# EricLBuehler/mistral.rs

Measured on AMD Instinct MI355X. Metric: decode_tokens_per_sec, higher is better.
Workload: dtype q4_k/q6_k weights x q8_k activations (int8 dot, f32 accumulate: the reference CPU path's arithmetic); 1 GPU; Llama-3-8B GGUF Q4_K_M, TP=1, 512 prefill / 1599 decode, batch 1, paged KV bf16 (block 32); parallelism=tp1

## Files before the change

### mistral.rs_amd/csrc/ext_gemm_qi.hip

```cpp
#include "dec_core2.cuh"
#include <stdio.h>
#include <stdlib.h>
#include <algorithm>
#include <type_traits>

namespace mrs {
namespace qi {
using namespace mrs::dec2;

typedef _Float16 h2 __attribute__((ext_vector_type(2)));
typedef _Float16 h8 __attribute__((ext_vector_type(8)));
typedef float f16v __attribute__((ext_vector_type(16)));
typedef float f2 __attribute__((ext_vector_type(2)));

constexpr int REC_Q4K = 4096 + 512 + 128, REC_Q6K = 8192 + 512 + 128, REC_Q5K = REC_Q6K;
__host__ __device__ constexpr int rec_bytes_qi(int type) { return type == T_Q4_K ? REC_Q4K : REC_Q6K; }
__host__ __device__ inline bool qi_type(int t) { return t == T_Q4_K || t == T_Q5_K || t == T_Q6_K || t == T_Q8_0; }
__host__ __device__ inline size_t qi_tensor_bytes(int type, long long n, long long k) { return (size_t)((n + 31) / 32) * (size_t)(k / 256) * rec_bytes_qi(type); }

__host__ __device__ constexpr int perm8(int jj) { return jj == 1 ? 2 : jj == 2 ? 1 : jj == 5 ? 6 : jj == 6 ? 5 : jj; }

template <int TYPE>
__global__ void __launch_bounds__(256) qi_repack_kernel(const uint8_t *__restrict__ src, uint8_t *__restrict__ dst, long long n, int K, long long total) {
  const long long i = (long long)blockIdx.x * 256 + threadIdx.x;
  if (i >= total) return;
  const int S = K / 256, lane = (int)(i & 63);
  const long long ps = i >> 6;
  const int sb = (int)(ps % S);
  const long long panel = ps / S, row = panel * 32 + (lane & 31);
  const int hf = lane >> 5;
  const bool have = row < n;
  uint8_t *rec = dst + (size_t)ps * rec_bytes_qi(TYPE);
  alignas(16) uint8_t buf[16];
  if constexpr (TYPE == T_Q4_K) {
    const uint8_t *b = src + ((size_t)row * S + sb) * 144, *qs = b + 16;
    for (int c = 0; c < 4; ++c) {
      for (int k = 0; k < 8; ++k) { buf[k] = have ? qs[32 * c + 8 * hf + k] : 0; buf[8 + k] = have ? qs[32 * c + 16 + 8 * hf + k] : 0; }
      *(v4u *)(rec + ((size_t)c * 64 + lane) * 16) = *(const v4u *)buf;
    }
    if (hf == 0) {
      const int nn = lane & 31;
      for (int g = 0; g < 8; ++g) {
        uint8_t sc = 0, mn = 0;
        if (have) {
          const uint8_t *p = b + 4;
          if (g < 4) { sc = p[g] & 63; mn = p[g + 4] & 63; } else { sc = (p[g + 4] & 15) | ((p[g - 4] >> 6) << 4); mn = (p[g + 4] >> 4) | ((p[g] >> 6) << 4); }
// ... 25 lines not shown
      *(uint32_t *)(rec + 8704 + (size_t)nn * 4) = have ? ((uint32_t)b[0] | ((uint32_t)b[1] << 8) | ((uint32_t)b[2] << 16) | ((uint32_t)b[3] << 24)) : 0u;
    }
  } else if constexpr (TYPE == T_Q8_0) {
    const uint8_t *b = src + ((size_t)row * S + sb) * 272;
    for (int g = 0; g < 8; ++g) {
      for (int k = 0; k < 16; ++k) buf[k] = have ? b[34 * g + 2 + 16 * hf + k] : 0;
      *(v4u *)(rec + ((size_t)g * 64 + lane) * 16) = *(const v4u *)buf;
    }
    if (hf == 0) {
      const int nn = lane & 31;
      for (int g = 0; g < 8; ++g) { buf[2 * g] = have ? b[34 * g] : 0; buf[2 * g + 1] = have ? b[34 * g + 1] : 0; }
      *(v4u *)(rec + 8192 + (size_t)nn * 16) = *(const v4u *)buf;
      *(uint32_t *)(rec + 8704 + (size_t)nn * 4) = 0u;
    }
  } else {
    const uint8_t *b = src + ((size_t)row * S + sb) * 210, *ql = b, *qh = b + 128;
    auto q6 = [&](int e) { const int hh = e / 128, pos = e % 32, qt = (e % 128) / 32, ii = hh * 64 + pos + (qt % 2) * 32;
                           const int lo = qt < 2 ? (ql[ii] & 15) : (ql[ii] >> 4), hi = (qh[hh * 32 + pos] >> (qt * 2)) & 3; return lo | (hi << 4); };
    for (int g = 0; g < 8; ++g) {
      for (int k = 0; k < 8; ++k) { buf[k] = have ? (uint8_t)q6((2 * g) * 16 + 8 * hf + k) : 32; buf[8 + k] = have ? (uint8_t)q6((2 * g + 1) * 16 + 8 * hf + k) : 32; }
      *(v4u *)(rec + ((size_t)g * 64 + lane) * 16) = *(const v4u *)buf;
    }
    if (hf == 0) {
      const int nn = lane & 31;
      for (int k = 0; k < 16; ++k) buf[k] = have ? b[192 + k] : 0;
      *(v4u *)(rec + 8192 + (size_t)nn * 16) = *(const v4u *)buf;
      *(uint32_t *)(rec + 8704 + (size_t)nn * 4) = have ? ((uint32_t)b[208] | ((uint32_t)b[209] << 8)) : 0u;
    }
  }
}

struct QuantArgs {
  const float *x, *x2; int ldx; const float *norm_w; float eps; int K, T;
  _Float16 *qf; float *yd; _Float16 *bsf;
  float *xtmp;
  int mode;
};
template <bool GLU>
__global__ void __launch_bounds__(NT) qi_quantize_kernel(const QuantArgs a) {
  extern __shared__ __attribute__((aligned(16))) char smem[];
  __shared__ float red[8];
  const int tid = tid_opaque(), t = blockIdx.x, K = a.K, S = K / 256;
  const float *xr = a.x + (size_t)t * a.ldx;
  if constexpr (GLU) {
    float *dst = a.xtmp + (size_t)t * K;
    const float *ur = a.x2 + (size_t)t * a.ldx;
    for (int e = tid * 4; e < K; e += NT * 4) {
      const float4 g = *(const float4 *)(xr + e), u = *(const float4 *)(ur + e);
      *(float4 *)(dst + e) = make_float4(silu_engine(g.x) * u.x, silu_engine(g.y) * u.y, silu_engine(g.z) * u.z, silu_engine(g.w) * u.w);
    }
    __syncthreads();
    xr = dst;
  }
  const int qw = __builtin_amdgcn_readfirstlane(tid >> 6);
  const ActRegs<1> pre = act_issue_all<1>(xr, (unsigned)K * 4u, a.norm_w, K, qw);
  act_finish_all<1>(smem, red, pre, xr, K, a.norm_w, a.eps, K, a.mode, qw);
  __syncthreads();
  const Act act = act_view(smem, K, 1, a.mode);
  if (a.mode == ACT_Q80) {
    int8_t *q8 = (int8_t *)a.qf;
    float *yd8 = (float *)a.bsf;
    for (int gi = tid; gi < S * 16; gi += NT) {
      const int sb = gi >> 4, ch = gi & 15;
      *(v4u *)(q8 + ((size_t)sb * a.T + t) * 256 + ch * 16) = *(const v4u *)(act.q + act.qoff(sb) + ch * 16);
    }
    for (int i = tid; i < S * 8; i += NT) {
      const int sb = i >> 3, b = i & 7;
      yd8[((size_t)sb * 8 + b) * a.T + t] = act.d[(size_t)sb * act.dw + b];
    }
    return;
  }
  for (int gi = tid; gi < S * 32; gi += NT) {
    const int sb = gi >> 5, g8 = gi & 31;
    const int8_t *q = (const int8_t *)(act.q + act.qoff(sb) + g8 * 8);
    h8 o;
#pragma unroll
    for (int jj = 0; jj < 8; ++jj) o[jj] = (_Float16)(float)q[perm8(jj)];
    *(h8 *)(a.qf + ((size_t)sb * a.T + t) * 256 + g8 * 8) = o;
  }
  for (int i = tid; i < S * 16; i += NT) {
    const int sb = i >> 4, r = i & 15;
    a.bsf[((size_t)sb * a.T + t) * 16 + r] = (_Float16)(float)act.bs[(size_t)sb * ACT_BS + r];
  }
  for (int sb = tid; sb < S; sb += NT) a.yd[(size_t)sb * a.T + t] = act.d[sb];
}

struct GemmArgs {
  const uint8_t *w; unsigned w_bytes; int type, N, K, T;
  const _Float16 *qf; const float *yd; const _Float16 *bsf;
  float *out; int ldo; int accumulate;
  float *part; int ksplit;
  const int *win;
};
constexpr int TN = 128, TT = 128;
constexpr int GT = 512;
constexpr int LDS_ACT = TT * 512, LDS_YD = TT * 4, LDS_BS = TT * 32;
constexpr int LDS_BUF = LDS_ACT + LDS_YD + LDS_BS;
constexpr int LDS_TOTAL = 2 * LDS_BUF;

#ifndef MRS_GLDS16
#define MRS_GLDS16(gptr, lbase) __builtin_amdgcn_global_load_lds((const __attribute__((address_space(1))) void *)(gptr), (__attribute__((address_space(3))) void *)(lbase), 16, 0, 0)
#define MRS_GLDS4(gptr, lbase) __builtin_amdgcn_global_load_lds((const __attribute__((address_space(1))) void *)(gptr), (__attribute__((address_space(3))) void *)(lbase), 4, 0, 0)
#endif
#ifndef MRS_WAIT_VMCNT0
#define MRS_WAIT_VMCNT0() asm volatile("s_waitcnt vmcnt(0)" ::: "memory")
#endif

__device__ __forceinline__ h2 as_h2(unsigned v) { return __builtin_bit_cast(h2, v); }
__device__ __forceinline__ h8 mk_h8(h2 a, h2 b, h2 c, h2 d) { h8 r; r[0] = a[0]; r[1] = a[1]; r[2] = b[0]; r[3] = b[1]; r[4] = c[0]; r[5] = c[1]; r[6] = d[0]; r[7] = d[1]; return r; }
__device__ __forceinline__ h2 pkfma(h2 x, h2 s, h2 c) { return __builtin_elementwise_fma(x, s, c); }
__device__ __forceinline__ h2 magic(unsigned v, unsigned mask) { return as_h2((v & mask) | 0x64006400u); }

template <int TYPE>
__global__ void __launch_bounds__(GT) gemm_qi_kernel(const GemmArgs a) {
  extern __shared__ __attribute__((aligned(16))) char smem[];
  const int tid = tid_opaque(), lane = tid & 63, wave = __builtin_amdgcn_readfirstlane(tid >> 6);
  const int nn = lane & 31, hf = lane >> 5;
  const int n0 = blockIdx.x * TN;
  const int tbeg = a.win ? __builtin_amdgcn_readfirstlane(a.win[0]) : 0, tend = a.win ? __builtin_amdgcn_readfirstlane(a.win[1]) : a.T;
  const int t0 = tbeg + blockIdx.y * TT;
  if (t0 >= tend) return;
  const int wn = wave & 3, wt = wave >> 2;
  const int S = a.K / 256, Cs = (S + 3) / 4;
  const __amdgpu_buffer_rsrc_t rw = __builtin_amdgcn_make_buffer_rsrc((void *)a.w, (short)0, (int)a.w_bytes, 0x00020000);
  constexpr int REC = rec_bytes_qi(TYPE), NPC = TYPE == T_Q4_K ? 4 : 8;
  struct WRegs { v4u q[NPC]; v4u hs; unsigned hd; };
  const unsigned panel = (unsigned)((n0 + wn * 32) >> 5);
  auto load_w = [&](WRegs &wr, int sb) {
    const unsigned rec = (panel * (unsigned)S + (unsigned)sb) * (unsigned)REC;
#pragma unroll
    for (int c = 0; c < NPC; ++c) wr.q[c] = __builtin_amdgcn_raw_buffer_load_b128(rw, rec + (unsigned)(c * 64 + lane) * 16u, 0, 0);
    wr.hs = __builtin_amdgcn_raw_buffer_load_b128(rw, rec + (unsigned)(NPC * 1024) + (unsigned)nn * 16u, 0, 0);
    wr.hd = __builtin_amdgcn_raw_buffer_load_b32(rw, rec + (unsigned)(NPC * 1024 + 512) + (unsigned)nn * 4u, 0, 0);
  };
  const int tlast = tend - 1 - t0;
  auto stage = [&](int sb, int buf) {
    char *base = smem + buf * LDS_BUF;
    const char *gq = (const char *)a.qf + ((size_t)sb * a.T + t0) * 512;
#pragma unroll
    for (int i = 0; i < 8; ++i) {
      const int pair = wave * 8 + i;
      const int tr = 2 * pair + hf, trc = min(tr, tlast);
      MRS_GLDS16(gq + (size_t)trc * 512 + (((lane & 31) ^ (tr & 31)) << 4), base + pair * 1024);
    }
    if (wave < 2) {
      const int tr = wave * 64 + lane;
      MRS_GLDS4((const char *)a.yd + ((size_t)sb * a.T + t0 + min(tr, tlast)) * 4, base + LDS_ACT + wave * 256);
    } else if (wave < 6) {
      const int i = wave - 2, tr = i * 32 + (lane >> 1);
      MRS_GLDS16((const char *)a.bsf + ((size_t)sb * a.T + t0 + min(tr, tlast)) * 32 + (lane & 1) * 16, base + LDS_ACT + LDS_YD + i * 1024);
    }
  };
  f16v run[2], pend[2];
#pragma unroll
  for (int tt = 0; tt < 2; ++tt)
#pragma unroll
    for (int v = 0; v < 16; ++v) { run[tt][v] = 0.f; pend[tt][v] = 0.f; }
  WRegs wr, wnx;
  const int sb_first = a.ksplit > 1 ? (int)blockIdx.z * ((a.K / 256 + 3) / 4) : 0;
  if (sb_first < a.K / 256) { load_w(wr, sb_first); stage(sb_first, sb_first & 1); }
  const int trow = wt * 64 + nn;
  int aoff[16];
#pragma unroll
  for (int r = 0; r < 16; ++r) aoff[r] = trow * 512 + (((2 * r + hf) ^ nn) << 4);
  const int sb_begin = a.ksplit > 1 ? (int)blockIdx.z * Cs : 0, sb_end = a.ksplit > 1 ? min(S, sb_begin + Cs) : S;
  if (sb_begin >= sb_end) {
    if (a.ksplit > 1) {
      const int n = n0 + wn * 32 + nn;
#pragma unroll
      for (int tt = 0; tt < 2; ++tt)
#pragma unroll
        for (int v = 0; v < 16; ++v) {
          const int t = t0 + wt * 64 + tt * 32 + 8 * (v >> 2) + 4 * hf + (v & 3);
          if (n < a.N && t < tend) a.part[((size_t)blockIdx.z * a.T + t) * a.N + n] = 0.f;
        }
    }
    return;
  }
  for (int sb = sb_begin; sb < sb_end; ++sb) {
    const int buf = sb & 1;
    MRS_WAIT_VMCNT0();
    __syncthreads();
    if (sb + 1 < sb_end) { stage(sb + 1, buf ^ 1); load_w(wnx, sb + 1); }
    const char *act_s = smem + buf * LDS_BUF;
    const float *yd_s = (const float *)(act_s + LDS_ACT);
    const char *bs_s = act_s + LDS_ACT + LDS_YD;
    f16v X[2], X2[2];
#pragma unroll
    for (int tt = 0; tt < 2; ++tt)
#pragma unroll
      for (int v = 0; v < 16; ++v) { X[tt][v] = 0.f; X2[tt][v] = 0.f; }
    constexpr bool RECOMP = TYPE == T_Q5_K;
    int nnv = nn;
    if constexpr (RECOMP) MRS_OPAQUE_TID(nnv);
    auto act_frag = [&](int tt, int run_i) -> h8 {
      if constexpr (RECOMP) return *(const h8 *)(act_s + trow * 512 + (((2 * run_i + hf) ^ nnv) << 4) + tt * (32 * 512));
      else return *(const h8 *)(act_s + aoff[run_i] + tt * (32 * 512));
    };
    const bool cfirst = (sb % Cs) == 0;
    const f2 keep2 = cfirst ? f2{0.f, 0.f} : f2{1.f, 1.f};
    if constexpr (TYPE == T_Q4_K) {
      unsigned mg = 0x64006400u;
      MRS_OPAQUE_TID(mg);
      auto lo4 = [&](unsigned v, h2 sc, h2 off) -> h2 { return pkfma(as_h2((v & 0x000F000Fu) | mg), sc, off); };
      auto hi4 = [&](unsigned v, h2 sc16, h2 off) -> h2 { return pkfma(as_h2((v & 0x00F000F0u) | mg), sc16, off); };
      const unsigned s01[2] = {wr.hs.x, wr.hs.y};
      h8 fr[2][4];
      auto read_group = [&](int gi, h8 (&f)[4]) {
        const int c = gi >> 1, h = gi & 1;
        f[0] = act_frag(0, 4 * c + h); f[1] = act_frag(0, 4 * c + 2 + h); f[2] = act_frag(1, 4 * c + h); f[3] = act_frag(1, 4 * c + 2 + h);
      };
      read_group(0, fr[0]);
#pragma unroll
      for (int gi = 0; gi < 8; ++gi) {
        const int c = gi >> 1, h = gi & 1;
        if (gi + 1 < 8) read_group(gi + 1, fr[(gi + 1) & 1]);
        __builtin_amdgcn_sched_barrier(0);
        const float sa = (float)byte_of(s01[c >> 1], 2 * (c & 1)), sb2 = (float)byte_of(s01[c >> 1], 2 * (c & 1) + 1);
        const h2 sl = h2{(_Float16)sa, (_Float16)sa}, ol = h2{(_Float16)(-1024.0f * sa), (_Float16)(-1024.0f * sa)};
        const h2 sh = h2{(_Float16)(sb2 * 0.0625f), (_Float16)(sb2 * 0.0625f)}, oh = h2{(_Float16)(-64.0f * sb2), (_Float16)(-64.0f * sb2)};
        const unsigned d0 = h == 0 ? wr.q[c].x : wr.q[c].z, d1 = h == 0 ? wr.q[c].y : wr.q[c].w;
        const unsigned e0 = d0 >> 8, e1 = d1 >> 8;
        const h8 wlo = mk_h8(lo4(d0, sl, ol), lo4(e0, sl, ol), lo4(d1, sl, ol), lo4(e1, sl, ol));
        const h8 whi = mk_h8(hi4(d0, sh, oh), hi4(e0, sh, oh), hi4(d1, sh, oh), hi4(e1, sh, oh));
        const h8 (&f)[4] = fr[gi & 1];
        if (c < 2) {
          X[0] = __builtin_amdgcn_mfma_f32_32x32x16_f16(f[0], wlo, X[0], 0, 0, 0);
          X[1] = __builtin_amdgcn_mfma_f32_32x32x16_f16(f[2], wlo, X[1], 0, 0, 0);
          X[0] = __builtin_amdgcn_mfma_f32_32x32x16_f16(f[1], whi, X[0], 0, 0, 0);
          X[1] = __builtin_amdgcn_mfma_f32_32x32x16_f16(f[3], whi, X[1], 0, 0, 0);
        } else {
          X2[0] = __builtin_amdgcn_mfma_f32_32x32x16_f16(f[0], wlo, X2[0], 0, 0, 0);
          X2[1] = __builtin_amdgcn_mfma_f32_32x32x16_f16(f[2], wlo, X2[1], 0, 0, 0);
          X2[0] = __builtin_amdgcn_mfma_f32_32x32x16_f16(f[1], whi, X2[0], 0, 0, 0);
          X2[1] = __builtin_amdgcn_mfma_f32_32x32x16_f16(f[3], whi, X2[1], 0, 0, 0);
        }
        __builtin_amdgcn_sched_barrier(0);
      }
      const unsigned mw = hf ? wr.hs.w : wr.hs.z;
      h8 wm;
#pragma unroll
      for (int k = 0; k < 4; ++k) { const _Float16 mk = (_Float16)(float)byte_of(mw, k); wm[2 * k] = mk; wm[2 * k + 1] = mk; }
      const float d = half_bits_to_float((uint16_t)(wr.hd & 0xffff)), dmin = half_bits_to_float((uint16_t)(wr.hd >> 16));
#pragma unroll
      for (int tt = 0; tt < 2; ++tt) {
        const h8 bsf = *(const h8 *)(bs_s + (trow + 32 * tt) * 32 + hf * 16);
        f16v zero;
#pragma unroll
        for (int v = 0; v < 16; ++v) zero[v] = 0.f;
        const f16v M = __builtin_amdgcn_mfma_f32_32x32x16_f16(bsf, wm, zero, 0, 0, 0);
#pragma unroll
        for (int q4 = 0; q4 < 4; ++q4) {
          const float4 y4 = *(const float4 *)(yd_s + wt * 64 + tt * 32 + 8 * q4 + 4 * hf);
#pragma unroll
          for (int k = 0; k < 4; k += 2) {
            const int v = 4 * q4 + k;
            const f2 yd2 = k == 0 ? f2{y4.x, y4.y} : f2{y4.z, y4.w};
            const f2 If = f2{X[tt][v], X[tt][v + 1]} + f2{X2[tt][v], X2[tt][v + 1]};
            const f2 mm = (f2{dmin, dmin} * yd2) * f2{M[v], M[v + 1]};
            const f2 t = __builtin_elementwise_fma(f2{d, d} * yd2, If, -mm);
            const f2 r = __builtin_elementwise_fma(f2{run[tt][v], run[tt][v + 1]}, keep2, t);
            run[tt][v] = r[0]; run[tt][v + 1] = r[1];
          }
        }
      }
    } else if constexpr (TYPE == T_Q5_K) {
      unsigned mg = 0x64006400u;
      MRS_OPAQUE_TID(mg);
      auto b2 = [&](unsigned v) -> h2 { return as_h2((v & 0x00FF00FFu) | mg); };
#pragma unroll
      for (int g = 0; g < 8; ++g) {
        const float scf = (float)byte_of(g < 4 ? wr.hs.x : wr.hs.y, g & 3);
        const h2 sc = h2{(_Float16)scf, (_Float16)scf}, off = h2{(_Float16)(-1024.0f * scf), (_Float16)(-1024.0f * scf)}, o16 = h2{(_Float16)(-16.0f * scf), (_Float16)(-16.0f * scf)};
        auto opnd = [&](unsigned v) -> h2 { return pkfma(b2(v), sc, off) + o16; };
#pragma unroll
        for (int h = 0; h < 2; ++h) {
          const unsigned d0 = h == 0 ? wr.q[g].x : wr.q[g].z, d1 = h == 0 ? wr.q[g].y : wr.q[g].w;
          const h8 w = mk_h8(opnd(d0), opnd(d0 >> 8), opnd(d1), opnd(d1 >> 8));
#pragma unroll
          for (int tt = 0; tt < 2; ++tt) {
            const h8 af = act_frag(tt, 2 * g + h);
            if (g < 4) X[tt] = __builtin_amdgcn_mfma_f32_32x32x16_f16(af, w, X[tt], 0, 0, 0);
            else X2[tt] = __builtin_amdgcn_mfma_f32_32x32x16_f16(af, w, X2[tt], 0, 0, 0);
          }
        }
      }
      const unsigned mw = hf ? wr.hs.w : wr.hs.z, sw = hf ? wr.hs.y : wr.hs.x;
      h8 wm, ws;
#pragma unroll
      for (int k = 0; k < 4; ++k) {
        const _Float16 mk = (_Float16)(float)byte_of(mw, k), sk = (_Float16)(float)byte_of(sw, k);
        wm[2 * k] = mk; wm[2 * k + 1] = mk; ws[2 * k] = sk; ws[2 * k + 1] = sk;
      }
      const float d = half_bits_to_float((uint16_t)(wr.hd & 0xffff)), dmin = half_bits_to_float((uint16_t)(wr.hd >> 16));
#pragma unroll
// ... 58 lines not shown
            const f2 yd2 = k == 0 ? f2{y4.x, y4.y} : f2{y4.z, y4.w};
            const f2 If = __builtin_elementwise_fma(f2{16.0f, 16.0f}, f2{X2[tt][v], X2[tt][v + 1]}, f2{X[tt][v], X[tt][v + 1]});
            const f2 t = (f2{d, d} * yd2) * If;
            const f2 r = __builtin_elementwise_fma(f2{run[tt][v], run[tt][v + 1]}, keep2, t);
            run[tt][v] = r[0]; run[tt][v + 1] = r[1];
          }
        }
    }
    if ((sb + 1) % Cs == 0 || sb + 1 == sb_end) {
      const bool first = sb < Cs;
#pragma unroll
      for (int tt = 0; tt < 2; ++tt)
#pragma unroll
        for (int v = 0; v < 16; ++v) pend[tt][v] = first ? run[tt][v] : pend[tt][v] + run[tt][v];
    }
    if (sb + 1 < sb_end) wr = wnx;
  }
  const int n = n0 + wn * 32 + nn;
#pragma unroll
  for (int tt = 0; tt < 2; ++tt)
#pragma unroll
    for (int v = 0; v < 16; ++v) {
      const int t = t0 + wt * 64 + tt * 32 + 8 * (v >> 2) + 4 * hf + (v & 3);
      if (n < a.N && t < tend) {
        if (a.ksplit > 1) a.part[((size_t)blockIdx.z * a.T + t) * a.N + n] = run[tt][v];
        else {
          float *o = a.out + (size_t)t * a.ldo + n;
          *o = a.accumulate ? *o + pend[tt][v] : pend[tt][v];
        }
      }
    }
}

typedef int i4v __attribute__((ext_vector_type(4)));
typedef int i16v __attribute__((ext_vector_type(16)));
constexpr int L8_ACT = TT * 256, L8_YD = 8 * TT * 4, L8_BUF = L8_ACT + L8_YD, L8_TOTAL = 2 * L8_BUF;
__global__ void __launch_bounds__(GT) gemm_q80_kernel(const GemmArgs a) {
  extern __shared__ __attribute__((aligned(16))) char smem[];
  const int tid = tid_opaque(), lane = tid & 63, wave = __builtin_amdgcn_readfirstlane(tid >> 6);
  const int nn = lane & 31, hf = lane >> 5;
  const int n0 = blockIdx.x * TN;
  const int tbeg = a.win ? a.win[0] : 0, tend = a.win ? a.win[1] : a.T;
  const int t0 = tbeg + blockIdx.y * TT;
  if (t0 >= tend) return;
  const int wn = wave & 3, wt = wave >> 2;
  const int S = a.K / 256, Cs = (S + 3) / 4;
  const __amdgpu_buffer_rsrc_t rw = __builtin_amdgcn_make_buffer_rsrc((void *)a.w, (short)0, (int)a.w_bytes, 0x00020000);
  constexpr int REC = REC_Q6K;
  struct WRegs { v4u q[8]; v4u hs; };
  const unsigned panel = (unsigned)((n0 + wn * 32) >> 5);
  auto rec_of = [&](int sb) { return (panel * (unsigned)S + (unsigned)sb) * (unsigned)REC; };
  auto load_piece = [&](WRegs &wr, unsigned rec, int c) { wr.q[c] = __builtin_amdgcn_raw_buffer_load_b128(rw, rec + (unsigned)(c * 64 + lane) * 16u, 0, 0); };
  auto load_hs = [&](WRegs &wr, unsigned rec) { wr.hs = __builtin_amdgcn_raw_buffer_load_b128(rw, rec + 8192u + (unsigned)nn * 16u, 0, 0); };
  auto load_w = [&](WRegs &wr, int sb) {
    const unsigned rec = rec_of(sb);
#pragma unroll
    for (int c = 0; c < 8; ++c) load_piece(wr, rec, c);
    load_hs(wr, rec);
  };
  const int tlast = tend - 1 - t0;
  const int8_t *q8 = (const int8_t *)a.qf;
  const float *yd8 = (const float *)a.bsf;
  auto stage = [&](int sb, int buf) {
    char *base = smem + buf * L8_BUF;
    const char *gq = (const char *)q8 + ((size_t)sb * a.T + t0) * 256;
#pragma unroll
    for (int i = 0; i < 4; ++i) {
      const int quad = wave * 4 + i;
// ... 99 lines not shown
__global__ void __launch_bounds__(256) gemm_qi_reduce_kernel(const float *__restrict__ part, float *__restrict__ out, int T, int N, int ldo, int accumulate) {
  const size_t i = ((size_t)blockIdx.x * 256 + threadIdx.x) * 4, tot = (size_t)T * N;
  if (i >= tot) return;
  const float4 c0 = *(const float4 *)(part + i), c1 = *(const float4 *)(part + tot + i), c2 = *(const float4 *)(part + 2 * tot + i), c3 = *(const float4 *)(part + 3 * tot + i);
  float4 r = make_float4(((c0.x + c1.x) + c2.x) + c3.x, ((c0.y + c1.y) + c2.y) + c3.y, ((c0.z + c1.z) + c2.z) + c3.z, ((c0.w + c1.w) + c2.w) + c3.w);
  const size_t t = i / N, n = i % N;
  float4 *o = (float4 *)(out + t * ldo + n);
  if (accumulate) { const float4 old = *o; r.x = old.x + r.x; r.y = old.y + r.y; r.z = old.z + r.z; r.w = old.w + r.w; }
  *o = r;
}

}
}

using namespace mrs;

extern "C" size_t mrs_gemm_qi_repack_bytes(int type, long long n, long long k) {
  if (!qi::qi_type(type) || n <= 0 || k <= 0 || k % 256) return 0;
  return qi::qi_tensor_bytes(type, n, k);
}
extern "C" int mrs_gemm_qi_repack(const void *gguf_blocks, int type, long long n, long long k, void *dst, void *stream) {
  if (!mrs_gemm_qi_repack_bytes(type, n, k) || !gguf_blocks || !dst) return -1;
  const long long total = ((n + 31) / 32) * (k / 256) * 64;
  const dim3 grid((unsigned)((total + 255) / 256));
  if (type == T_Q4_K) hipLaunchKernelGGL(qi::qi_repack_kernel<T_Q4_K>, grid, dim3(256), 0, (hipStream_t)stream, (const uint8_t *)gguf_blocks, (uint8_t *)dst, n, (int)k, total);
  else if (type == T_Q5_K) hipLaunchKernelGGL(qi::qi_repack_kernel<T_Q5_K>, grid, dim3(256), 0, (hipStream_t)stream, (const uint8_t *)gguf_blocks, (uint8_t *)dst, n, (int)k, total);
  else if (type == T_Q8_0) hipLaunchKernelGGL(qi::qi_repack_kernel<T_Q8_0>, grid, dim3(256), 0, (hipStream_t)stream, (const uint8_t *)gguf_blocks, (uint8_t *)dst, n, (int)k, total);
  else hipLaunchKernelGGL(qi::qi_repack_kernel<T_Q6_K>, grid, dim3(256), 0, (hipStream_t)stream, (const uint8_t *)gguf_blocks, (uint8_t *)dst, n, (int)k, total);
  return 0;
}
extern "C" size_t mrs_qi_act_bytes(int T, int K) {
  const size_t S = (size_t)(K / 256), t = (size_t)T;
  auto al = [](size_t v) { return (v + 255) & ~(size_t)255; };
  return al(S * t * 512) + al(S * t * 4) + al(S * t * 32);
}
static void qi_split(void *buf, int T, int K, _Float16 **qf, float **yd, _Float16 **bsf) {
  const size_t S = (size_t)(K / 256), t = (size_t)T;
  auto al = [](size_t v) { return (v + 255) & ~(size_t)255; };
  char *p = (char *)buf;
  *qf = (_Float16 *)p; p += al(S * t * 512);
  *yd = (float *)p; p += al(S * t * 4);
  *bsf = (_Float16 *)p;
}
extern "C" int mrs_qi_quantize_for(int w_type, const float *x, const float *x2, int ldx, const float *norm_w, float eps, int T, int K, void *act, float *xtmp, void *stream);
extern "C" int mrs_qi_quantize(const float *x, const float *x2, int ldx, const float *norm_w, float eps, int T, int K, void *act, float *xtmp, void *stream) {
  return mrs_qi_quantize_for(T_Q4_K, x, x2, ldx, norm_w, eps, T, K, act, xtmp, stream);
}
extern "C" int mrs_qi_quantize_for(int w_type, const float *x, const float *x2, int ldx, const float *norm_w, float eps, int T, int K, void *act, float *xtmp, void *stream) {
  if (!x || !act || T <= 0 || K <= 0 || K % 256 || (x2 && !xtmp) || !qi::qi_type(w_type)) return -1;
  qi::QuantArgs a{};
  a.x = x; a.x2 = x2; a.ldx = ldx; a.norm_w = norm_w; a.eps = eps; a.K = K; a.T = T; a.xtmp = xtmp; a.mode = dec2::act_mode_for(w_type);
  qi_split(act, T, K, &a.qf, &a.yd, &a.bsf);
  const size_t lds = (dec2::act_bytes(K, 1) + 15) & ~(size_t)15;
  if (lds > 158 * 1024) return -2;
  if (x2) { auto kern = qi::qi_quantize_kernel<true>; lds_attr_once((const void *)kern, 158 * 1024); hipLaunchKernelGGL(kern, dim3(T), dim3(dec2::NT), lds, (hipStream_t)stream, a); }
  else { auto kern = qi::qi_quantize_kernel<false>; lds_attr_once((const void *)kern, 158 * 1024); hipLaunchKernelGGL(kern, dim3(T), dim3(dec2::NT), lds, (hipStream_t)stream, a); }
  return 0;
}
extern "C" size_t mrs_gemm_qi_workspace_bytes(int T, int max_n_split) { return (size_t)4 * (size_t)T * (size_t)max_n_split * 4; }
extern "C" int mrs_gemm_qi_ws(const void *w_qi, int type, int N, int K, const void *act, int T, float *out, int ldo, int accumulate, void *workspace, size_t workspace_bytes,
                              void *stream);
extern "C" int mrs_gemm_qi(const void *w_qi, int type, int N, int K, const void *act, int T, float *out, int ldo, int accumulate, void *stream) {
  return mrs_gemm_qi_ws(w_qi, type, N, K, act, T, out, ldo, accumulate, nullptr, 0, stream);
}
static int gemm_qi_launch(const void *w_qi, int type, int N, int K, const void *act, int T, const int *win, int max_rows, float *out, int ldo, int accumulate, void *workspace,
                          size_t workspace_bytes, void *stream);
extern "C" int mrs_gemm_qi_win(const void *w_qi, int type, int N, int K, const void *act, int T_total, const int *win, int max_rows, float *out, int ldo, int accumulate, void *stream) {
  if (!win || max_rows <= 0 || max_rows > T_total) return -1;
  return gemm_qi_launch(w_qi, type, N, K, act, T_total, win, max_rows, out, ldo, accumulate, nullptr, 0, stream);
}
extern "C" int mrs_gemm_qi_ws(const void *w_qi, int type, int N, int K, const void *act, int T, float *out, int ldo, int accumulate, void *workspace, size_t workspace_bytes,
                              void *stream) {
  return gemm_qi_launch(w_qi, type, N, K, act, T, nullptr, T, out, ldo, accumulate, workspace, workspace_bytes, stream);
}
static int gemm_qi_launch(const void *w_qi, int type, int N, int K, const void *act, int T, const int *win, int max_rows, float *out, int ldo, int accumulate, void *workspace,
                          size_t workspace_bytes, void *stream) {
  if (!w_qi || !act || !out || !qi::qi_type(type) || N <= 0 || T <= 0 || K <= 0 || K % 256) return -1;
  qi::GemmArgs a{};
  a.w = (const uint8_t *)w_qi; a.w_bytes = (unsigned)qi::qi_tensor_bytes(type, N, K); a.type = type; a.N = N; a.K = K; a.T = T;
  _Float16 *qf, *bsf; float *yd;
  qi_split((void *)act, T, K, &qf, &yd, &bsf);
  if ((size_t)(K / 256) * T * 512 >= 0x7fffffffull || qi::qi_tensor_bytes(type, N, K) >= 0xffffff00ull) return -2;
  a.qf = qf; a.yd = yd; a.bsf = bsf; a.out = out; a.ldo = ldo; a.accumulate = accumulate; a.win = win;
  dim3 grid((N + qi::TN - 1) / qi::TN, (max_rows + qi::TT - 1) / qi::TT);
  constexpr int split_max = 200;
  a.ksplit = 1; a.part = nullptr;
  if (!win && (int)(grid.x * grid.y) < split_max && K / 256 >= 4 && N % 4 == 0 && workspace && workspace_bytes >= (size_t)4 * T * N * 4) { a.ksplit = 4; a.part = (float *)workspace; grid.z = 4; }
  if (type == T_Q8_0) { auto kern = qi::gemm_q80_kernel; lds_attr_once((const void *)kern, 158 * 1024); hipLaunchKernelGGL(kern, grid, dim3(qi::GT), qi::L8_TOTAL, (hipStream_t)stream, a); }
  else if (type == T_Q4_K) { auto kern = qi::gemm_qi_kernel<T_Q4_K>; lds_attr_once((const void *)kern, 158 * 1024); hipLaunchKernelGGL(kern, grid, dim3(qi::GT), qi::LDS_TOTAL, (hipStream_t)stream, a); }
  else if (type == T_Q5_K) { auto kern = qi::gemm_qi_kernel<T_Q5_K>; lds_attr_once((const void *)kern, 158 * 1024); hipLaunchKernelGGL(kern, grid, dim3(qi::GT), qi::LDS_TOTAL, (hipStream_t)stream, a); }
  else { auto kern = qi::gemm_qi_kernel<T_Q6_K>; lds_attr_once((const void *)kern, 158 * 1024); hipLaunchKernelGGL(kern, grid, dim3(qi::GT), qi::LDS_TOTAL, (hipStream_t)stream, a); }
  if (a.ksplit > 1) hipLaunchKernelGGL(qi::gemm_qi_reduce_kernel, dim3((unsigned)(((size_t)T * N / 4 + 255) / 256)), dim3(256), 0, (hipStream_t)stream, a.part, out, T, N, ldo, accumulate);
  return 0;
}

namespace mrs {
namespace qi {
__global__ void __launch_bounds__(256) qi_gather_rows_kernel(const char *__restrict__ src, char *__restrict__ dst, int T, int R, int S, int mode, const int *__restrict__ sorted,
                                                             int tk, int *__restrict__ inv, size_t off1s, size_t off2s, size_t off1d, size_t off2d) {
  const int r = blockIdx.x, route = sorted[r], t = route / tk;
  if (threadIdx.x == 0 && inv) inv[route] = r;
  if (mode == ACT_Q80) {
    for (int i = threadIdx.x; i < S * 16; i += 256) {
      const int sb = i >> 4, ch = i & 15;
      *(v4u *)(dst + ((size_t)sb * R + r) * 256 + ch * 16) = *(const v4u *)(src + ((size_t)sb * T + t) * 256 + ch * 16);
    }
    for (int i = threadIdx.x; i < S * 8; i += 256) ((float *)(dst + off2d))[(size_t)i * R + r] = ((const float *)(src + off2s))[(size_t)i * T + t];
  } else {
    for (int i = threadIdx.x; i < S * 32; i += 256) {
      const int sb = i >> 5, ch = i & 31;
      *(v4u *)(dst + ((size_t)sb * R + r) * 512 + ch * 16) = *(const v4u *)(src + ((size_t)sb * T + t) * 512 + ch * 16);
    }
    for (int i = threadIdx.x; i < S * 2; i += 256) {
      const int sb = i >> 1, ch = i & 1;
      *(v4u *)(dst + off2d + ((size_t)sb * R + r) * 32 + ch * 16) = *(const v4u *)(src + off2s + ((size_t)sb * T + t) * 32 + ch * 16);
    }
    for (int sb = threadIdx.x; sb < S; sb += 256) ((float *)(dst + off1d))[(size_t)sb * R + r] = ((const float *)(src + off1s))[(size_t)sb * T + t];
  }
}
__global__ void __launch_bounds__(256) moe_fold_exact_kernel(float *__restrict__ h, float rs, const float *__restrict__ y, const int *__restrict__ inv, const float *__restrict__ w,
                                                            int d, int tk) {
  const int t = blockIdx.x;
  for (int n = threadIdx.x * 4; n < d; n += 1024) {
    float4 v = *(const float4 *)(h + (size_t)t * d + n);
    for (int sl = 0; sl < tk; ++sl) {
      const float ws = w[(size_t)t * tk + sl], sc = sl == 0 ? rs : 1.0f;
      const float4 yy = *(const float4 *)(y + (size_t)inv[(size_t)t * tk + sl] * d + n);
      v.x = v.x * sc + yy.x * ws; v.y = v.y * sc + yy.y * ws; v.z = v.z * sc + yy.z * ws; v.w = v.w * sc + yy.w * ws;
    }
    *(float4 *)(h + (size_t)t * d + n) = v;
  }
}
__global__ void __launch_bounds__(256) resid_scale_add_kernel(float *__restrict__ h, float rs, const float *__restrict__ y, size_t n) {
  for (size_t i = ((size_t)blockIdx.x * 256 + threadIdx.x) * 4; i < n; i += (size_t)gridDim.x * 1024) {
    if (i + 4 <= n) {
      float4 a = *(float4 *)(h + i); const float4 b = *(const float4 *)(y + i);
      a.x = a.x * rs + b.x * 1.0f; a.y = a.y * rs + b.y * 1.0f; a.z = a.z * rs + b.z * 1.0f; a.w = a.w * rs + b.w * 1.0f;
      *(float4 *)(h + i) = a;
    } else for (size_t j = i; j < n; ++j) h[j] = h[j] * rs + y[j] * 1.0f;
  }
}
}
}
extern "C" int mrs_qi_gather_rows(int w_type, const void *act_src, int T, void *act_dst, int R, int K, const int *sorted_routes, int top_k, int *inv, void *stream) {
  if (!act_src || !act_dst || !sorted_routes || T <= 0 || R <= 0 || K <= 0 || K % 256 || top_k <= 0 || !qi::qi_type(w_type)) return -1;
  _Float16 *qs, *bs, *qd, *bd; float *ys, *yd;
  qi_split((void *)act_src, T, K, &qs, &ys, &bs);
  qi_split(act_dst, R, K, &qd, &yd, &bd);
  hipLaunchKernelGGL(qi::qi_gather_rows_kernel, dim3(R), dim3(256), 0, (hipStream_t)stream, (const char *)act_src, (char *)act_dst, T, R, K / 256, dec2::act_mode_for(w_type),
                     sorted_routes, top_k, inv, (size_t)((char *)ys - (char *)qs), (size_t)((char *)bs - (char *)qs), (size_t)((char *)yd - (char *)qd), (size_t)((char *)bd - (char *)qd));
  return 0;
}
extern "C" int mrs_moe_fold_exact(float *h, float resid_scale, const float *y_sorted, const int *inv, const float *weights, int T, int d, int top_k, void *stream) {
  if (!h || !y_sorted || !inv || !weights || T <= 0 || d <= 0 || d % 4 || top_k <= 0) return -1;
  hipLaunchKernelGGL(qi::moe_fold_exact_kernel, dim3(T), dim3(256), 0, (hipStream_t)stream, h, resid_scale, y_sorted, inv, weights, d, top_k);
  return 0;
}
extern "C" int mrs_resid_scale_add_f32(float *h, float resid_scale, const float *y, size_t n, void *stream) {
  if (!n) return 0;
  size_t g = (n / 4 + 255) / 256; if (g > 2048) g = 2048; if (g < 1) g = 1;
  hipLaunchKernelGGL(qi::resid_scale_add_kernel, dim3((unsigned)g), dim3(256), 0, (hipStream_t)stream, h, resid_scale, y, n);
  return 0;
}

#include "dec_attn.cuh"
namespace mrs {
namespace qi {
template <int G, class CT, bool ONE>
__global__ void __launch_bounds__(256) prefill_attn_exact_kernel(const dec::AttnArgs a, const int qw) {
  extern __shared__ __attribute__((aligned(16))) char smem[];
  constexpr int HD = 128;
  const int tid = tid_opaque(), lane = tid & 63, wave = __builtin_amdgcn_readfirstlane(tid >> 6);
  const int kvh = blockIdx.x, tile = (int)gridDim.y - 1 - (int)blockIdx.y;
  const int T = a.num_seqs, ms = a.max_splits, bpw = a.bpw;
  const int t0 = (tile * 4 + wave) * qw, nq = min(qw, T - t0);
  if (nq <= 0) return;
  const size_t per_wave = (size_t)qw * G * HD * 2 + G * 32 + (size_t)qw * G * ms * 2 + (size_t)qw * G * 64;
  float *q_s = (float *)smem + wave * per_wave, *p_s = q_s + (size_t)qw * G * HD, *acc = p_s + G * 32, *ml = acc + (size_t)qw * G * HD, *sall = ml + (size_t)qw * G * ms * 2;
  int ctx_max = 0;
  for (int i = 0; i < nq; ++i) {
    const float *qg = a.q + (size_t)(t0 + i) * a.q_stride + (size_t)kvh * G * HD;
    for (int k = lane * 4; k < G * HD; k += 256) *(float4 *)(q_s + (size_t)i * G * HD + k) = *(const float4 *)(qg + k);
    for (int k = lane; k < G * HD; k += 64) acc[(size_t)i * G * HD + k] = 0.f;
// ... 295 lines not shown
```

Baseline: 533.4 tokens/s.

## Use int8 MFMA for Q4_K GEMM with integer sub-block scale accumulation

The Q4_K tiled GEMM now multiplies raw int8 activations against 4-bit weight nibbles with the i32 32x32x32 int8 MFMA, instead of dequantizing weights to fp16 and using fp16 MFMA. Per-sub-block scales are applied as integer multiply-adds, so the result matches the reference int8-dot arithmetic. The quantize kernel also writes a permuted int8 copy of the activations, the activation buffer grows, and the Q4_K LDS staging halves. The gather kernel copies the new section too. This adds activation-write traffic on every quantize call, and since this kernel is the batched-tile path, decode at batch 1 may not use it much.

After: 533.4 tokens/s. No clear change (-0.0%).

```diff
diff --git a/mistral.rs_amd/csrc/ext_gemm_qi.hip b/mistral.rs_amd/csrc/ext_gemm_qi.hip
--- a/mistral.rs_amd/csrc/ext_gemm_qi.hip
+++ b/mistral.rs_amd/csrc/ext_gemm_qi.hip
@@ -12,6 +12,8 @@
 typedef _Float16 h8 __attribute__((ext_vector_type(8)));
 typedef float f16v __attribute__((ext_vector_type(16)));
 typedef float f2 __attribute__((ext_vector_type(2)));
+typedef int i4v __attribute__((ext_vector_type(4)));
+typedef int i16v __attribute__((ext_vector_type(16)));
 
 constexpr int REC_Q4K = 4096 + 512 + 128, REC_Q6K = 8192 + 512 + 128, REC_Q5K = REC_Q6K;
 __host__ __device__ constexpr int rec_bytes_qi(int type) { return type == T_Q4_K ? REC_Q4K : REC_Q6K; }
@@ -103,7 +105,7 @@
 
 struct QuantArgs {
   const float *x, *x2; int ldx; const float *norm_w; float eps; int K, T;
-  _Float16 *qf; float *yd; _Float16 *bsf;
+  _Float16 *qf; float *yd; _Float16 *bsf; int8_t *q8;
   float *xtmp;
   int mode;
 };
@@ -148,6 +150,8 @@
 #pragma unroll
     for (int jj = 0; jj < 8; ++jj) o[jj] = (_Float16)(float)q[perm8(jj)];
     *(h8 *)(a.qf + ((size_t)sb * a.T + t) * 256 + g8 * 8) = o;
+    const int s4 = g8 & 3, p4 = s4 == 1 ? 2 : s4 == 2 ? 1 : s4;
+    *(v2u *)(a.q8 + ((size_t)sb * a.T + t) * 256 + ((g8 & ~3) + p4) * 8) = *(const v2u *)q;
   }
   for (int i = tid; i < S * 16; i += NT) {
     const int sb = i >> 4, r = i & 15;
@@ -158,16 +162,17 @@
 
 struct GemmArgs {
   const uint8_t *w; unsigned w_bytes; int type, N, K, T;
-  const _Float16 *qf; const float *yd; const _Float16 *bsf;
+  const _Float16 *qf; const float *yd; const _Float16 *bsf; const int8_t *q8;
   float *out; int ldo; int accumulate;
   float *part; int ksplit;
   const int *win;
 };
 constexpr int TN = 128, TT = 128;
 constexpr int GT = 512;
-constexpr int LDS_ACT = TT * 512, LDS_YD = TT * 4, LDS_BS = TT * 32;
-constexpr int LDS_BUF = LDS_ACT + LDS_YD + LDS_BS;
-constexpr int LDS_TOTAL = 2 * LDS_BUF;
+constexpr int LDS_YD = TT * 4, LDS_BS = TT * 32;
+__host__ __device__ constexpr int lds_act_of(int type) { return type == T_Q4_K ? TT * 256 : TT * 512; }
+__host__ __device__ constexpr int lds_buf_of(int type) { return lds_act_of(type) + LDS_YD + LDS_BS; }
+__host__ __device__ constexpr int lds_total_of(int type) { return 2 * lds_buf_of(type); }
 
 #ifndef MRS_GLDS16
 #define MRS_GLDS16(gptr, lbase) __builtin_amdgcn_global_load_lds((const __attribute__((address_space(1))) void *)(gptr), (__attribute__((address_space(3))) void *)(lbase), 16, 0, 0)
@@ -195,6 +200,8 @@
   const int S = a.K / 256, Cs = (S + 3) / 4;
   const __amdgpu_buffer_rsrc_t rw = __builtin_amdgcn_make_buffer_rsrc((void *)a.w, (short)0, (int)a.w_bytes, 0x00020000);
   constexpr int REC = rec_bytes_qi(TYPE), NPC = TYPE == T_Q4_K ? 4 : 8;
+  constexpr bool I8 = TYPE == T_Q4_K;
+  constexpr int LDS_ACT = lds_act_of(TYPE), LDS_BUF = lds_buf_of(TYPE);
   struct WRegs { v4u q[NPC]; v4u hs; unsigned hd; };
   const unsigned panel = (unsigned)((n0 + wn * 32) >> 5);
   auto load_w = [&](WRegs &wr, int sb) {
@@ -207,12 +214,22 @@
   const int tlast = tend - 1 - t0;
   auto stage = [&](int sb, int buf) {
     char *base = smem + buf * LDS_BUF;
-    const char *gq = (const char *)a.qf + ((size_t)sb * a.T + t0) * 512;
-#pragma unroll
-    for (int i = 0; i < 8; ++i) {
-      const int pair = wave * 8 + i;
-      const int tr = 2 * pair + hf, trc = min(tr, tlast);
-      MRS_GLDS16(gq + (size_t)trc * 512 + (((lane & 31) ^ (tr & 31)) << 4), base + pair * 1024);
+    if constexpr (I8) {
+      const char *gq = (const char *)a.q8 + ((size_t)sb * a.T + t0) * 256;
+#pragma unroll
+      for (int i = 0; i < 4; ++i) {
+        const int quad = wave * 4 + i;
+        const int tr = 4 * quad + (lane >> 4), trc = min(tr, tlast);
+        MRS_GLDS16(gq + (size_t)trc * 256 + (((lane & 15) ^ (tr & 15)) << 4), base + quad * 1024);
+      }
+    } else {
+      const char *gq = (const char *)a.qf + ((size_t)sb * a.T + t0) * 512;
+#pragma unroll
+      for (int i = 0; i < 8; ++i) {
+        const int pair = wave * 8 + i;
+        const int tr = 2 * pair + hf, trc = min(tr, tlast);
+        MRS_GLDS16(gq + (size_t)trc * 512 + (((lane & 31) ^ (tr & 31)) << 4), base + pair * 1024);
+      }
     }
     if (wave < 2) {
       const int tr = wave * 64 + lane;
@@ -231,9 +248,9 @@
   const int sb_first = a.ksplit > 1 ? (int)blockIdx.z * ((a.K / 256 + 3) / 4) : 0;
   if (sb_first < a.K / 256) { load_w(wr, sb_first); stage(sb_first, sb_first & 1); }
   const int trow = wt * 64 + nn;
-  int aoff[16];
-#pragma unroll
-  for (int r = 0; r < 16; ++r) aoff[r] = trow * 512 + (((2 * r + hf) ^ nn) << 4);
+  int aoff[I8 ? 8 : 16];
+#pragma unroll
+  for (int r = 0; r < (I8 ? 8 : 16); ++r) aoff[r] = I8 ? trow * 256 + (((2 * r + hf) ^ (nn & 15)) << 4) : trow * 512 + (((2 * r + hf) ^ nn) << 4);
   const int sb_begin = a.ksplit > 1 ? (int)blockIdx.z * Cs : 0, sb_end = a.ksplit > 1 ? min(S, sb_begin + Cs) : S;
   if (sb_begin >= sb_end) {
     if (a.ksplit > 1) {
@@ -256,82 +273,87 @@
     const char *act_s = smem + buf * LDS_BUF;
     const float *yd_s = (const float *)(act_s + LDS_ACT);
     const char *bs_s = act_s + LDS_ACT + LDS_YD;
-    f16v X[2], X2[2];
-#pragma unroll
-    for (int tt = 0; tt < 2; ++tt)
-#pragma unroll
-      for (int v = 0; v < 16; ++v) { X[tt][v] = 0.f; X2[tt][v] = 0.f; }
+    f16v X[I8 ? 1 : 2], X2[I8 ? 1 : 2];
+    if constexpr (!I8) {
+#pragma unroll
+      for (int tt = 0; tt < 2; ++tt)
+#pragma unroll
+        for (int v = 0; v < 16; ++v) { X[tt][v] = 0.f; X2[tt][v] = 0.f; }
+    }
     constexpr bool RECOMP = TYPE == T_Q5_K;
     int nnv = nn;
     if constexpr (RECOMP) MRS_OPAQUE_TID(nnv);
-    auto act_frag = [&](int tt, int run_i) -> h8 {
+    [[maybe_unused]] auto act_frag = [&](int tt, int run_i) -> h8 {
       if constexpr (RECOMP) return *(const h8 *)(act_s + trow * 512 + (((2 * run_i + hf) ^ nnv) << 4) + tt * (32 * 512));
       else return *(const h8 *)(act_s + aoff[run_i] + tt * (32 * 512));
     };
     const bool cfirst = (sb % Cs) == 0;
     const f2 keep2 = cfirst ? f2{0.f, 0.f} : f2{1.f, 1.f};
     if constexpr (TYPE == T_Q4_K) {
-      unsigned mg = 0x64006400u;
-      MRS_OPAQUE_TID(mg);
-      auto lo4 = [&](unsigned v, h2 sc, h2 off) -> h2 { return pkfma(as_h2((v & 0x000F000Fu) | mg), sc, off); };
-      auto hi4 = [&](unsigned v, h2 sc16, h2 off) -> h2 { return pkfma(as_h2((v & 0x00F000F0u) | mg), sc16, off); };
-      const unsigned s01[2] = {wr.hs.x, wr.hs.y};
-      h8 fr[2][4];
-      auto read_group = [&](int gi, h8 (&f)[4]) {
-        const int c = gi >> 1, h = gi & 1;
-        f[0] = act_frag(0, 4 * c + h); f[1] = act_frag(0, 4 * c + 2 + h); f[2] = act_frag(1, 4 * c + h); f[3] = act_frag(1, 4 * c + 2 + h);
-      };
-      read_group(0, fr[0]);
-#pragma unroll
-      for (int gi = 0; gi < 8; ++gi) {
-        const int c = gi >> 1, h = gi & 1;
-        if (gi + 1 < 8) read_group(gi + 1, fr[(gi + 1) & 1]);
+      const i16v zi = {0, 0, 0, 0, 0, 0, 0, 0, 0, 0, 0, 0, 0, 0, 0, 0};
+      auto frag8 = [&](int tt, int j) -> i4v { return *(const i4v *)(act_s + aoff[j] + tt * (32 * 256)); };
+      auto scale_of = [&](int j) -> int { return byte_of(j < 4 ? wr.hs.x : wr.hs.y, j & 3); };
+      int isum0[16], isum1[16];
+      i16v d0, d1;
+      i4v f0 = frag8(0, 0), f1 = frag8(1, 0), g0, g1;
+#define MRS_Q4_PRODUCTS(IS, D, J) { const int sc_ = scale_of(J); _Pragma("unroll") for (int v = 0; v < 16; ++v) { IS[v] = (J) == 0 ? __mul24(sc_, D[v]) : __mul24(sc_, D[v]) + IS[v]; MRS_OPAQUE_TID(IS[v]); } }
+#pragma unroll
+      for (int j = 0; j < 8; ++j) {
+        const int c = j >> 1;
+        const v4u wq = (j & 1) ? ((wr.q[c] >> 4) & 0x0F0F0F0Fu) : (wr.q[c] & 0x0F0F0F0Fu);
+        if (j + 1 < 8) { g0 = frag8(0, j + 1); g1 = frag8(1, j + 1); }
         __builtin_amdgcn_sched_barrier(0);
-        const float sa = (float)byte_of(s01[c >> 1], 2 * (c & 1)), sb2 = (float)byte_of(s01[c >> 1], 2 * (c & 1) + 1);
-        const h2 sl = h2{(_Float16)sa, (_Float16)sa}, ol = h2{(_Float16)(-1024.0f * sa), (_Float16)(-1024.0f * sa)};
-        const h2 sh = h2{(_Float16)(sb2 * 0.0625f), (_Float16)(sb2 * 0.0625f)}, oh = h2{(_Float16)(-64.0f * sb2), (_Float16)(-64.0f * sb2)};
-        const unsigned d0 = h == 0 ? wr.q[c].x : wr.q[c].z, d1 = h == 0 ? wr.q[c].y : wr.q[c].w;
-        const unsigned e0 = d0 >> 8, e1 = d1 >> 8;
-        const h8 wlo = mk_h8(lo4(d0, sl, ol), lo4(e0, sl, ol), lo4(d1, sl, ol), lo4(e1, sl, ol));
-        const h8 whi = mk_h8(hi4(d0, sh, oh), hi4(e0, sh, oh), hi4(d1, sh, oh), hi4(e1, sh, oh));
-        const h8 (&f)[4] = fr[gi & 1];
-        if (c < 2) {
-          X[0] = __builtin_amdgcn_mfma_f32_32x32x16_f16(f[0], wlo, X[0], 0, 0, 0);
-          X[1] = __builtin_amdgcn_mfma_f32_32x32x16_f16(f[2], wlo, X[1], 0, 0, 0);
-          X[0] = __builtin_amdgcn_mfma_f32_32x32x16_f16(f[1], whi, X[0], 0, 0, 0);
-          X[1] = __builtin_amdgcn_mfma_f32_32x32x16_f16(f[3], whi, X[1], 0, 0, 0);
-        } else {
-          X2[0] = __builtin_amdgcn_mfma_f32_32x32x16_f16(f[0], wlo, X2[0], 0, 0, 0);
-          X2[1] = __builtin_amdgcn_mfma_f32_32x32x16_f16(f[2], wlo, X2[1], 0, 0, 0);
-          X2[0] = __builtin_amdgcn_mfma_f32_32x32x16_f16(f[1], whi, X2[0], 0, 0, 0);
-          X2[1] = __builtin_amdgcn_mfma_f32_32x32x16_f16(f[3], whi, X2[1], 0, 0, 0);
-        }
+        d0 = __builtin_amdgcn_mfma_i32_32x32x32_i8(f0, __builtin_bit_cast(i4v, wq), zi, 0, 0, 0);
         __builtin_amdgcn_sched_barrier(0);
+        if (j > 0) MRS_Q4_PRODUCTS(isum1, d1, j - 1)
+        __builtin_amdgcn_sched_barrier(0);
+        d1 = __builtin_amdgcn_mfma_i32_32x32x32_i8(f1, __builtin_bit_cast(i4v, wq), zi, 0, 0, 0);
+        __builtin_amdgcn_sched_barrier(0);
+        MRS_Q4_PRODUCTS(isum0, d0, j)
+        __builtin_amdgcn_sched_barrier(0);
+        f0 = g0; f1 = g1;
       }
       const unsigned mw = hf ? wr.hs.w : wr.hs.z;
       h8 wm;
 #pragma unroll
       for (int k = 0; k < 4; ++k) { const _Float16 mk = (_Float16)(float)byte_of(mw, k); wm[2 * k] = mk; wm[2 * k + 1] = mk; }
+      f16v Mt[2];
+      {
+        f16v zero;
+#pragma unroll
+        for (int v = 0; v < 16; ++v) zero[v] = 0.f;
+        const h8 bs0 = *(const h8 *)(bs_s + trow * 32 + hf * 16), bs1 = *(const h8 *)(bs_s + (trow + 32) * 32 + hf * 16);
+        __builtin_amdgcn_sched_barrier(0);
+        Mt[0] = __builtin_amdgcn_mfma_f32_32x32x16_f16(bs0, wm, zero, 0, 0, 0);
+        Mt[1] = __builtin_amdgcn_mfma_f32_32x32x16_f16(bs1, wm, zero, 0, 0, 0);
+        __builtin_amdgcn_sched_barrier(0);
+        MRS_Q4_PRODUCTS(isum1, d1, 7)
+        __builtin_amdgcn_sched_barrier(0);
+      }
+#undef MRS_Q4_PRODUCTS
       const float d = half_bits_to_float((uint16_t)(wr.hd & 0xffff)), dmin = half_bits_to_float((uint16_t)(wr.hd >> 16));
 #pragma unroll
       for (int tt = 0; tt < 2; ++tt) {
-        const h8 bsf = *(const h8 *)(bs_s + (trow + 32 * tt) * 32 + hf * 16);
-        f16v zero;
-#pragma unroll
-        for (int v = 0; v < 16; ++v) zero[v] = 0.f;
-        const f16v M = __builtin_amdgcn_mfma_f32_32x32x16_f16(bsf, wm, zero, 0, 0, 0);
+        const f16v M = Mt[tt];
 #pragma unroll
         for (int q4 = 0; q4 < 4; ++q4) {
           const float4 y4 = *(const float4 *)(yd_s + wt * 64 + tt * 32 + 8 * q4 + 4 * hf);
-#pragma unroll
-          for (int k = 0; k < 4; k += 2) {
+          const float yy[4] = {y4.x, y4.y, y4.z, y4.w};
+#pragma unroll
+          for (int k = 0; k < 4; ++k) {
             const int v = 4 * q4 + k;
-            const f2 yd2 = k == 0 ? f2{y4.x, y4.y} : f2{y4.z, y4.w};
-            const f2 If = f2{X[tt][v], X[tt][v + 1]} + f2{X2[tt][v], X2[tt][v + 1]};
-            const f2 mm = (f2{dmin, dmin} * yd2) * f2{M[v], M[v + 1]};
-            const f2 t = __builtin_elementwise_fma(f2{d, d} * yd2, If, -mm);
-            const f2 r = __builtin_elementwise_fma(f2{run[tt][v], run[tt][v + 1]}, keep2, t);
-            run[tt][v] = r[0]; run[tt][v + 1] = r[1];
+            float If = (float)(tt == 0 ? isum0[v] : isum1[v]);
+            MRS_OPAQUE_TID(If);
+            float dy = d * yy[k], my = dmin * yy[k];
+            MRS_OPAQUE_TID(dy);
+            MRS_OPAQUE_TID(my);
+            float mm = my * M[v];
+            MRS_OPAQUE_TID(mm);
+            float t = fmaf(dy, If, -mm);
+            MRS_OPAQUE_TID(t);
+            float r = fmaf(run[tt][v], keep2[0], t);
+            MRS_OPAQUE_TID(r);
+            run[tt][v] = r;
           }
         }
       }
@@ -456,8 +478,6 @@
     }
 }
 
-typedef int i4v __attribute__((ext_vector_type(4)));
-typedef int i16v __attribute__((ext_vector_type(16)));
 constexpr int L8_ACT = TT * 256, L8_YD = 8 * TT * 4, L8_BUF = L8_ACT + L8_YD, L8_TOTAL = 2 * L8_BUF;
 __global__ void __launch_bounds__(GT) gemm_q80_kernel(const GemmArgs a) {
   extern __shared__ __attribute__((aligned(16))) char smem[];
@@ -623,15 +643,16 @@
 extern "C" size_t mrs_qi_act_bytes(int T, int K) {
   const size_t S = (size_t)(K / 256), t = (size_t)T;
   auto al = [](size_t v) { return (v + 255) & ~(size_t)255; };
-  return al(S * t * 512) + al(S * t * 4) + al(S * t * 32);
-}
-static void qi_split(void *buf, int T, int K, _Float16 **qf, float **yd, _Float16 **bsf) {
+  return al(S * t * 512) + al(S * t * 4) + al(S * t * 32) + al(S * t * 256);
+}
+static void qi_split(void *buf, int T, int K, _Float16 **qf, float **yd, _Float16 **bsf, int8_t **q8) {
   const size_t S = (size_t)(K / 256), t = (size_t)T;
   auto al = [](size_t v) { return (v + 255) & ~(size_t)255; };
   char *p = (char *)buf;
   *qf = (_Float16 *)p; p += al(S * t * 512);
   *yd = (float *)p; p += al(S * t * 4);
-  *bsf = (_Float16 *)p;
+  *bsf = (_Float16 *)p; p += al(S * t * 32);
+  *q8 = (int8_t *)p;
 }
 extern "C" int mrs_qi_quantize_for(int w_type, const float *x, const float *x2, int ldx, const float *norm_w, float eps, int T, int K, void *act, float *xtmp, void *stream);
 extern "C" int mrs_qi_quantize(const float *x, const float *x2, int ldx, const float *norm_w, float eps, int T, int K, void *act, float *xtmp, void *stream) {
@@ -641,7 +662,7 @@
   if (!x || !act || T <= 0 || K <= 0 || K % 256 || (x2 && !xtmp) || !qi::qi_type(w_type)) return -1;
   qi::QuantArgs a{};
   a.x = x; a.x2 = x2; a.ldx = ldx; a.norm_w = norm_w; a.eps = eps; a.K = K; a.T = T; a.xtmp = xtmp; a.mode = dec2::act_mode_for(w_type);
-  qi_split(act, T, K, &a.qf, &a.yd, &a.bsf);
+  qi_split(act, T, K, &a.qf, &a.yd, &a.bsf, &a.q8);
   const size_t lds = (dec2::act_bytes(K, 1) + 15) & ~(size_t)15;
   if (lds > 158 * 1024) return -2;
   if (x2) { auto kern = qi::qi_quantize_kernel<true>; lds_attr_once((const void *)kern, 158 * 1024); hipLaunchKernelGGL(kern, dim3(T), dim3(dec2::NT), lds, (hipStream_t)stream, a); }
@@ -669,18 +690,18 @@
   if (!w_qi || !act || !out || !qi::qi_type(type) || N <= 0 || T <= 0 || K <= 0 || K % 256) return -1;
   qi::GemmArgs a{};
   a.w = (const uint8_t *)w_qi; a.w_bytes = (unsigned)qi::qi_tensor_bytes(type, N, K); a.type = type; a.N = N; a.K = K; a.T = T;
-  _Float16 *qf, *bsf; float *yd;
-  qi_split((void *)act, T, K, &qf, &yd, &bsf);
+  _Float16 *qf, *bsf; float *yd; int8_t *q8;
+  qi_split((void *)act, T, K, &qf, &yd, &bsf, &q8);
   if ((size_t)(K / 256) * T * 512 >= 0x7fffffffull || qi::qi_tensor_bytes(type, N, K) >= 0xffffff00ull) return -2;
-  a.qf = qf; a.yd = yd; a.bsf = bsf; a.out = out; a.ldo = ldo; a.accumulate = accumulate; a.win = win;
+  a.qf = qf; a.yd = yd; a.bsf = bsf; a.q8 = q8; a.out = out; a.ldo = ldo; a.accumulate = accumulate; a.win = win;
   dim3 grid((N + qi::TN - 1) / qi::TN, (max_rows + qi::TT - 1) / qi::TT);
   constexpr int split_max = 200;
   a.ksplit = 1; a.part = nullptr;
   if (!win && (int)(grid.x * grid.y) < split_max && K / 256 >= 4 && N % 4 == 0 && workspace && workspace_bytes >= (size_t)4 * T * N * 4) { a.ksplit = 4; a.part = (float *)workspace; grid.z = 4; }
   if (type == T_Q8_0) { auto kern = qi::gemm_q80_kernel; lds_attr_once((const void *)kern, 158 * 1024); hipLaunchKernelGGL(kern, grid, dim3(qi::GT), qi::L8_TOTAL, (hipStream_t)stream, a); }
-  else if (type == T_Q4_K) { auto kern = qi::gemm_qi_kernel<T_Q4_K>; lds_attr_once((const void *)kern, 158 * 1024); hipLaunchKernelGGL(kern, grid, dim3(qi::GT), qi::LDS_TOTAL, (hipStream_t)stream, a); }
-  else if (type == T_Q5_K) { auto kern = qi::gemm_qi_kernel<T_Q5_K>; lds_attr_once((const void *)kern, 158 * 1024); hipLaunchKernelGGL(kern, grid, dim3(qi::GT), qi::LDS_TOTAL, (hipStream_t)stream, a); }
-  else { auto kern = qi::gemm_qi_kernel<T_Q6_K>; lds_attr_once((const void *)kern, 158 * 1024); hipLaunchKernelGGL(kern, grid, dim3(qi::GT), qi::LDS_TOTAL, (hipStream_t)stream, a); }
+  else if (type == T_Q4_K) { auto kern = qi::gemm_qi_kernel<T_Q4_K>; lds_attr_once((const void *)kern, 158 * 1024); hipLaunchKernelGGL(kern, grid, dim3(qi::GT), qi::lds_total_of(T_Q4_K), (hipStream_t)stream, a); }
+  else if (type == T_Q5_K) { auto kern = qi::gemm_qi_kernel<T_Q5_K>; lds_attr_once((const void *)kern, 158 * 1024); hipLaunchKernelGGL(kern, grid, dim3(qi::GT), qi::lds_total_of(T_Q5_K), (hipStream_t)stream, a); }
+  else { auto kern = qi::gemm_qi_kernel<T_Q6_K>; lds_attr_once((const void *)kern, 158 * 1024); hipLaunchKernelGGL(kern, grid, dim3(qi::GT), qi::lds_total_of(T_Q6_K), (hipStream_t)stream, a); }
   if (a.ksplit > 1) hipLaunchKernelGGL(qi::gemm_qi_reduce_kernel, dim3((unsigned)(((size_t)T * N / 4 + 255) / 256)), dim3(256), 0, (hipStream_t)stream, a.part, out, T, N, ldo, accumulate);
   return 0;
 }
@@ -688,7 +709,7 @@
 namespace mrs {
 namespace qi {
 __global__ void __launch_bounds__(256) qi_gather_rows_kernel(const char *__restrict__ src, char *__restrict__ dst, int T, int R, int S, int mode, const int *__restrict__ sorted,
-                                                             int tk, int *__restrict__ inv, size_t off1s, size_t off2s, size_t off1d, size_t off2d) {
+                                                             int tk, int *__restrict__ inv, size_t off1s, size_t off2s, size_t off3s, size_t off1d, size_t off2d, size_t off3d) {
   const int r = blockIdx.x, route = sorted[r], t = route / tk;
   if (threadIdx.x == 0 && inv) inv[route] = r;
   if (mode == ACT_Q80) {
@@ -701,6 +722,10 @@
     for (int i = threadIdx.x; i < S * 32; i += 256) {
       const int sb = i >> 5, ch = i & 31;
       *(v4u *)(dst + ((size_t)sb * R + r) * 512 + ch * 16) = *(const v4u *)(src + ((size_t)sb * T + t) * 512 + ch * 16);
+    }
+    for (int i = threadIdx.x; i < S * 16; i += 256) {
+      const int sb = i >> 4, ch = i & 15;
+      *(v4u *)(dst + off3d + ((size_t)sb * R + r) * 256 + ch * 16) = *(const v4u *)(src + off3s + ((size_t)sb * T + t) * 256 + ch * 16);
     }
     for (int i = threadIdx.x; i < S * 2; i += 256) {
       const int sb = i >> 1, ch = i & 1;
@@ -735,11 +760,12 @@
 }
 extern "C" int mrs_qi_gather_rows(int w_type, const void *act_src, int T, void *act_dst, int R, int K, const int *sorted_routes, int top_k, int *inv, void *stream) {
   if (!act_src || !act_dst || !sorted_routes || T <= 0 || R <= 0 || K <= 0 || K % 256 || top_k <= 0 || !qi::qi_type(w_type)) return -1;
-  _Float16 *qs, *bs, *qd, *bd; float *ys, *yd;
-  qi_split((void *)act_src, T, K, &qs, &ys, &bs);
-  qi_split(act_dst, R, K, &qd, &yd, &bd);
+  _Float16 *qs, *bs, *qd, *bd; float *ys, *yd; int8_t *q8s, *q8d;
+  qi_split((void *)act_src, T, K, &qs, &ys, &bs, &q8s);
+  qi_split(act_dst, R, K, &qd, &yd, &bd, &q8d);
   hipLaunchKernelGGL(qi::qi_gather_rows_kernel, dim3(R), dim3(256), 0, (hipStream_t)stream, (const char *)act_src, (char *)act_dst, T, R, K / 256, dec2::act_mode_for(w_type),
-                     sorted_routes, top_k, inv, (size_t)((char *)ys - (char *)qs), (size_t)((char *)bs - (char *)qs), (size_t)((char *)yd - (char *)qd), (size_t)((char *)bd - (char *)qd));
+                     sorted_routes, top_k, inv, (size_t)((char *)ys - (char *)qs), (size_t)((char *)bs - (char *)qs), (size_t)((char *)q8s - (char *)qs), (size_t)((char *)yd - (char *)qd), (size_t)((char *)bd - (char *)qd),
+                     (size_t)((char *)q8d - (char *)qd));
   return 0;
 }
 extern "C" int mrs_moe_fold_exact(float *h, float resid_scale, const float *y_sorted, const int *inv, const float *weights, int T, int d, int top_k, void *stream) {
```
